# hrz2000/CustomNeRF

Hardware: AMD Instinct MI355X
Metric: training rays/s (higher is better)
Workload: dtype f16

## Files before the change

customnerf_amd/csrc/field.hip:

```cpp
#include "field_common.h"

template <bool H>
__device__ __forceinline__ void fld_stage_all(typename Prec<H>::elem_t *lds, const FieldDims &dm, const FieldLds &lo, const float *__restrict__ pnet,
                                              const float *__restrict__ pden, const float *__restrict__ prgb, bool with_rgb,
                                              uint32_t i0 = threadIdx.x, uint32_t istride = FLD_THREADS) {
    using P = Prec<H>;
    const uint32_t S64 = FLD_HID / P::KS, Senc = dm.enc_pad / P::KS;
    const float *n0 = pnet, *n1 = pnet + FLD_HID * dm.enc_pad;
    const float *n2 = n1 + (dm.n_hidden_geo == 2 ? FLD_HID * FLD_HID : 0);
    fld_stage_layer<H, 0>(lds + lo.off[0], n0, FLD_HID, dm.enc_pad, 2, Senc, dm.enc_pad, i0, istride);
    if (dm.n_hidden_geo == 2) fld_stage_layer<H, 1>(lds + lo.off[1], n1, FLD_HID, FLD_HID, 2, S64, FLD_HID, i0, istride);
    fld_stage_layer<H, 1>(lds + lo.off[2], n2, FLD_HID, FLD_HID, 2, S64, FLD_HID, i0, istride);
    fld_stage_layer<H, 1>(lds + lo.off[3], pden, FLD_HID, FLD_HID, 2, S64, FLD_HID, i0, istride);
    fld_stage_layer<H, 1>(lds + lo.off[4], pden + FLD_HID * FLD_HID, 16, FLD_HID, 1, S64, FLD_HID, i0, istride);
    if (with_rgb) {
        const uint32_t in_r0 = FLD_HID + FLD_DIR;
        fld_stage_layer<H, 2>(lds + lo.off[5], prgb, FLD_HID, in_r0, 2, in_r0 / P::KS, in_r0, i0, istride);
        fld_stage_layer<H, 1>(lds + lo.off[6], prgb + FLD_HID * in_r0, 16, FLD_HID, 1, S64, FLD_HID, i0, istride);
    }
}

__global__ void __launch_bounds__(FLD_THREADS) k_field_pack(_Float16 *__restrict__ img, FieldDims dm, const float *__restrict__ pnet,
                                                            const float *__restrict__ pden, const float *__restrict__ prgb) {
    const FieldLds lo = fld_lds_layout<true>(dm);
    fld_stage_all<true>(img, dm, lo, pnet, pden, prgb, true, blockIdx.x * FLD_THREADS + threadIdx.x, gridDim.x * FLD_THREADS);
}
__device__ __forceinline__ void fld_copy_image(_Float16 *lds, const void *__restrict__ img, uint32_t n_halves) {
    const uint4 *src = reinterpret_cast<const uint4 *>(img);
    uint4 *dst = reinterpret_cast<uint4 *>(lds);
    for (uint32_t c = threadIdx.x; c < n_halves / 8; c += FLD_THREADS) dst[c] = src[c];
}

template <bool H, bool RELU>
__device__ __forceinline__ void fld_c_to_b(const cn_f16v (&acc)[2], typename Prec<H>::frag_t *b) {
    using P = Prec<H>;
#pragma unroll
    for (int u = 0; u < 2; u++) {
#pragma unroll
        for (int sub = 0; sub < P::FR; sub++) {
            if constexpr (H) {
                union { cn_h8 h; cn_h2 p[4]; } f;
#pragma unroll
                for (int j = 0; j < 4; j++) {
                    cn_h2 v = {(_Float16)acc[u][8 * sub + 2 * j], (_Float16)acc[u][8 * sub + 2 * j + 1]};
                    if (RELU) v = __builtin_elementwise_max(v, cn_h2{(_Float16)0, (_Float16)0});
                    f.p[j] = v;
                }
                b[u * P::FR + sub] = f.h;
            } else {
                float v = acc[u][sub];
                if (RELU) v = fmaxf(v, 0.0f);
                b[u * P::FR + sub] = v;
            }
        }
    }
}

template <bool H>
__device__ __forceinline__ void fld_dir_frags(const float *__restrict__ dirs, uint32_t dir_group, uint32_t p, bool valid, uint32_t hi,
                                              typename Prec<H>::frag_t *b) {
    float dx = 0, dy = 0, dz = 0;
    if (valid) {
        const float *d = dirs + (size_t)(p / dir_group) * 3;
        dx = d[0]; dy = d[1]; dz = d[2];
    }
    fld_dir_frags_from<H>(dx, dy, dz, true, hi, b);
}

__device__ __forceinline__ float fld_round_half(float v) { return (float)(_Float16)v; }

template <bool H, int SENC, int NGEO>
__global__ void __launch_bounds__(FLD_THREADS, H ? 2 : 1) k_field_fwd(const void *__restrict__ enc, const float *__restrict__ xyz, const float *__restrict__ dirs,
                                                           uint32_t dir_group, uint32_t P_, FieldDims dm, const float *__restrict__ pnet,
                                                           const float *__restrict__ pden, const float *__restrict__ prgb,
                                                           float *__restrict__ sigma, float *__restrict__ rgbc, uint32_t enc_stride,
                                                           const void *__restrict__ wimg) {
    using PR = Prec<H>;
    using frag_t = typename PR::frag_t;
    extern __shared__ __attribute__((aligned(16))) unsigned char fld_lds[];
    typename PR::elem_t *wl = reinterpret_cast<typename PR::elem_t *>(fld_lds);
    const FieldLds lo = fld_lds_layout<H>(dm);
    const bool with_rgb = rgbc != nullptr;
#ifdef CNERF_TUNING
    const bool nostage = (dir_group >> 31) != 0;
    dir_group &= 0x7FFFFFFFu;
    if (nostage) { fld_stage_all<H>(wl, dm, lo, pnet, pden, prgb, with_rgb); __syncthreads(); }
#endif
    if constexpr (H) {
        if (wimg) fld_copy_image(wl, wimg, with_rgb ? lo.off[7] : lo.off[5]);
        else fld_stage_all<H>(wl, dm, lo, pnet, pden, prgb, with_rgb);
    } else {
        fld_stage_all<H>(wl, dm, lo, pnet, pden, prgb, with_rgb);
    }
    __syncthreads();

    const uint32_t lane = threadIdx.x & 63, wave = threadIdx.x >> 6, hi = lane >> 5;
    constexpr uint32_t S64 = FLD_HID / PR::KS, SDIR = FLD_DIR / PR::KS;
    const uint32_t n_tiles = (P_ + FLD_TILE - 1) / FLD_TILE;
    unsigned char *dir_scratch = fld_lds + lo.off[7] * sizeof(typename PR::elem_t) + wave * 64;
    const bool dir_uniform = H && (dir_group % FLD_TILE) == 0;
    for (uint32_t tile = blockIdx.x * FLD_WAVES + wave; tile < n_tiles; tile += gridDim.x * FLD_WAVES) {
        asm volatile("" ::: "memory");
        const uint32_t p = tile * FLD_TILE + (lane & 31);
        const bool valid = p < P_;

        frag_t x0[SENC];
        fld_load_enc<H, SENC>(enc, enc_stride, dm.L, p, valid, hi, x0);

        cn_f16v acc[2];
        frag_t h[2 * PR::FR];
        fld_zero(acc);
        fld_gemm<H, 2, SENC>(wl + lo.off[0], SENC, 0, x0, lane, acc);
        fld_c_to_b<H, true>(acc, h);
        if (NGEO == 2) {
            fld_zero(acc);
            fld_gemm<H, 2, S64>(wl + lo.off[1], S64, 0, h, lane, acc);
            fld_c_to_b<H, true>(acc, h);
        }
        frag_t fea[2 * PR::FR];
        fld_zero(acc);
        fld_gemm<H, 2, S64>(wl + lo.off[2], S64, 0, h, lane, acc);
        fld_c_to_b<H, false>(acc, fea);

        fld_zero(acc);
        fld_gemm<H, 2, S64>(wl + lo.off[3], S64, 0, fea, lane, acc);
        fld_c_to_b<H, true>(acc, h);
        cn_f16v out[1];
        fld_zero(out);
        fld_gemm<H, 1, S64>(wl + lo.off[4], S64, 0, h, lane, out);
        if (valid && hi == 0) {
            float raw = out[0][0];
            if (H) raw = fld_round_half(raw);
            const float x = xyz[(size_t)p * 3], y = xyz[(size_t)p * 3 + 1], z = xyz[(size_t)p * 3 + 2];
            const float g = H ? 5.0f * __expf(-(x * x + y * y + z * z) * (1.0f / 0.08f)) : 5.0f * expf(-(x * x + y * y + z * z) / 0.08f);
            sigma[p] = H ? __expf(raw + g) : expf(raw + g);
        }

        if (with_rgb) {
            frag_t dfr[SDIR];
            if constexpr (H) {
                if (dir_uniform) {
                    const float *dp = dirs + (size_t)(__builtin_amdgcn_readfirstlane(tile) * FLD_TILE / dir_group) * 3;
                    fld_dir_frags_uniform(dp[0], dp[1], dp[2], lane, hi, dir_scratch, dfr);
                } else {
                    fld_dir_frags<H>(dirs, dir_group, p, valid, hi, dfr);
                }
            } else {
                fld_dir_frags<H>(dirs, dir_group, p, valid, hi, dfr);
            }
            constexpr uint32_t SR0 = S64 + SDIR;
            fld_zero(acc);
            fld_gemm<H, 2, S64>(wl + lo.off[5], SR0, 0, fea, lane, acc);
            fld_gemm<H, 2, SDIR>(wl + lo.off[5], SR0, S64, dfr, lane, acc);
            fld_c_to_b<H, true>(acc, h);
            fld_zero(out);
            fld_gemm<H, 1, S64>(wl + lo.off[6], S64, 0, h, lane, out);
            if (valid && hi == 0) {
                float o4[4];
#pragma unroll
                for (int k = 0; k < 4; k++) {
                    float v = H ? __builtin_amdgcn_rcpf(1.0f + __expf(-out[0][k])) : 1.0f / (1.0f + expf(-out[0][k]));
                    if (H) v = fld_round_half(v);
                    o4[k] = (k < (int)dm.n_rgb_out) ? v : 0.0f;
                }
                *reinterpret_cast<float4 *>(rgbc + (size_t)p * 4) = make_float4(o4[0], o4[1], o4[2], o4[3]);
            }
        }
    }
}

template <bool H>
static int fld_launch_fwd(const void *enc, const float *xyz, const float *dirs, uint32_t dir_group, uint32_t P_, const FieldDims &dm,
                          const float *pnet, const float *pden, const float *prgb, float *sigma, float *rgbc, hipStream_t st, uint32_t enc_stride,
                          const void *wimg) {
    const FieldLds lo = fld_lds_layout<H>(dm);
    const uint32_t lds_bytes = lo.off[7] * sizeof(typename Prec<H>::elem_t) + FLD_WAVES * 64;
    const uint32_t n_tiles = cn_div_up(P_, FLD_TILE);
    uint32_t blocks = cn_div_up(n_tiles, FLD_WAVES);
    const uint32_t max_blocks = H ? 768 : 256;
    if (blocks > max_blocks) blocks = max_blocks;
#ifdef CNERF_TUNING
    static const int nostage = cn_tune_env("CNERF_FLD_NOSTAGE", 0);
    if (nostage) dir_group |= 0x80000000u;
#endif
    const bool ok = fld_dispatch(dm, [&](auto se16, auto ng) {
        auto kern = k_field_fwd<H, se16 * 16 / Prec<H>::KS, ng>;
        (void)hipFuncSetAttribute(reinterpret_cast<const void *>(kern), hipFuncAttributeMaxDynamicSharedMemorySize, lds_bytes);
        hipLaunchKernelGGL(kern, dim3(blocks), dim3(FLD_THREADS), lds_bytes, st, enc, xyz, dirs, dir_group, P_, dm, pnet, pden, prgb, sigma, rgbc, enc_stride, wimg);
    });
    if (!ok) return CNERF_EINVAL;
    return cn_launch_status();
}

extern "C" {

int cnerf_field_weight_image_bytes(uint32_t enc_dim, uint32_t n_hidden_geo, uint32_t n_rgb_out, uint64_t *bytes) {
    FieldDims dm;
    int rc = fld_dims(enc_dim, n_hidden_geo, n_rgb_out, dm);
    if (rc) return rc;
    if (!bytes) return CNERF_ENULL;
    *bytes = (uint64_t)fld_lds_layout<true>(dm).off[7] * sizeof(_Float16);
    return CNERF_OK;
}

int cnerf_field_pack_weights(uint32_t enc_dim, uint32_t n_hidden_geo, uint32_t n_rgb_out, const float *params_net, const float *params_den,
                             const float *params_rgb, void *image, uint64_t image_bytes, void *stream) {
    FieldDims dm;
    int rc = fld_dims(enc_dim, n_hidden_geo, n_rgb_out, dm);
    if (rc) return rc;
    if (!params_net || !params_den || !params_rgb || !image) return CNERF_ENULL;
    const uint32_t n = fld_lds_layout<true>(dm).off[7];
    if ((((uintptr_t)image) & 15) || image_bytes < (uint64_t)n * sizeof(_Float16)) return CNERF_EINVAL;
    hipLaunchKernelGGL(k_field_pack, dim3(cn_div_up(n, 4 * FLD_THREADS)), dim3(FLD_THREADS), 0, CN_STREAM(stream), reinterpret_cast<_Float16 *>(image), dm,
                       params_net, params_den, params_rgb);
    return cn_launch_status();
}

int cnerf_field_forward_img(const void *enc, const float *xyz, const float *dirs, uint32_t dir_group, uint32_t P_, uint32_t enc_dim,
                            uint32_t n_hidden_geo, uint32_t n_rgb_out, const float *params_net, const float *params_den, const float *params_rgb,
                            float *sigma, float *rgbc, int dtype, uint32_t enc_level_stride, const void *weight_image, void *stream) {
    FieldDims dm;
    int rc = fld_dims(enc_dim, n_hidden_geo, n_rgb_out, dm);
    if (rc) return rc;
    if (dtype != CNERF_F32 && dtype != CNERF_F16) return CNERF_EINVAL;
    if (dtype != CNERF_F16) weight_image = nullptr;
    if (((uintptr_t)weight_image) & 15) return CNERF_EINVAL;
    if (enc_level_stride == 0) enc_level_stride = P_;
    if (enc_level_stride < P_) return CNERF_EINVAL;
    if (P_ == 0) return CNERF_OK;
    if (!enc || !xyz || !params_net || !params_den || !sigma) return CNERF_ENULL;
    if (rgbc && (!dirs || !params_rgb || dir_group == 0)) return CNERF_ENULL;
    if (rgbc && (((uintptr_t)rgbc) & 15)) return CNERF_EINVAL;
    if (dtype == CNERF_F16)
        return fld_launch_fwd<true>(enc, xyz, dirs, dir_group, P_, dm, params_net, params_den, params_rgb, sigma, rgbc, CN_STREAM(stream), enc_level_stride,
                                    weight_image);
    return fld_launch_fwd<false>(enc, xyz, dirs, dir_group, P_, dm, params_net, params_den, params_rgb, sigma, rgbc, CN_STREAM(stream), enc_level_stride,
                                 nullptr);
}

int cnerf_field_forward_strided(const void *enc, const float *xyz, const float *dirs, uint32_t dir_group, uint32_t P_, uint32_t enc_dim,
                                uint32_t n_hidden_geo, uint32_t n_rgb_out, const float *params_net, const float *params_den, const float *params_rgb,
                                float *sigma, float *rgbc, int dtype, uint32_t enc_level_stride, void *stream) {
    return cnerf_field_forward_img(enc, xyz, dirs, dir_group, P_, enc_dim, n_hidden_geo, n_rgb_out, params_net, params_den, params_rgb, sigma, rgbc, dtype,
                                   enc_level_stride, nullptr, stream);
}

int cnerf_field_forward(const void *enc, const float *xyz, const float *dirs, uint32_t dir_group, uint32_t P_, uint32_t enc_dim,
                        uint32_t n_hidden_geo, uint32_t n_rgb_out, const float *params_net, const float *params_den, const float *params_rgb,
                        float *sigma, float *rgbc, int dtype, void *stream) {
    return cnerf_field_forward_strided(enc, xyz, dirs, dir_group, P_, enc_dim, n_hidden_geo, n_rgb_out, params_net, params_den, params_rgb, sigma, rgbc, dtype,
                                       P_, stream);
}

}
```

Measured before the change: 8.914 million.

## Process two point tiles per wave in field forward to reuse weight fragments

The forward field kernel now has each wave handle NT tiles at once (two when the encoding is f16 and small). Each weight fragment read from LDS feeds MFMAs for both tiles, and all global inputs (encoding, xyz, dirs) are loaded up front with clamped indices so their latency overlaps. This cuts LDS weight traffic per point and exposes more independent MFMA work. In exchange it doubles accumulator and fragment register use, which may lower occupancy, and it halves the number of wave work items at the same grid cap.

```diff
diff --git a/customnerf_amd/csrc/field.hip b/customnerf_amd/csrc/field.hip
--- a/customnerf_amd/csrc/field.hip
+++ b/customnerf_amd/csrc/field.hip
@@ -56,18 +56,74 @@
     }
 }
 
-template <bool H>
-__device__ __forceinline__ void fld_dir_frags(const float *__restrict__ dirs, uint32_t dir_group, uint32_t p, bool valid, uint32_t hi,
-                                              typename Prec<H>::frag_t *b) {
-    float dx = 0, dy = 0, dz = 0;
-    if (valid) {
-        const float *d = dirs + (size_t)(p / dir_group) * 3;
-        dx = d[0]; dy = d[1]; dz = d[2];
-    }
-    fld_dir_frags_from<H>(dx, dy, dz, true, hi, b);
-}
-
 __device__ __forceinline__ float fld_round_half(float v) { return (float)(_Float16)v; }
+
+template <bool H, int SENC>
+struct FldTileIn {
+    typename std::conditional<H, uint32_t, float>::type e[H ? 4 * SENC : SENC];
+    float x[3], d[3];
+};
+
+template <bool H, int SENC>
+__device__ __forceinline__ void fld_load_tile(const void *__restrict__ enc, uint32_t enc_stride, uint32_t L, const float *__restrict__ xyz,
+                                              const float *__restrict__ dirs, uint32_t dir_group, uint32_t tile, uint32_t n_tiles, uint32_t P_,
+                                              uint32_t lane, FldTileIn<H, SENC> &in) {
+    const uint32_t hi = lane >> 5;
+    const uint32_t tc = tile < n_tiles ? tile : n_tiles - 1;
+    const uint32_t pl = tc * FLD_TILE + (lane & 31), pc = pl < P_ ? pl : P_ - 1;
+    if constexpr (H) {
+        const uint32_t *e = reinterpret_cast<const uint32_t *>(enc);
+#pragma unroll
+        for (int i = 0; i < 4 * SENC; i++) {
+            const uint32_t level = 8 * (i >> 2) + 4 * hi + (i & 3);
+            in.e[i] = e[(size_t)(level < L ? level : L - 1) * enc_stride + pc];
+        }
+    } else {
+        const float *e = reinterpret_cast<const float *>(enc);
+#pragma unroll
+        for (int s = 0; s < SENC; s++) {
+            const uint32_t feat = 2 * s + hi, level = feat >> 1;
+            in.e[s] = e[((size_t)(level < L ? level : L - 1) * enc_stride + pc) * 2 + (feat & 1)];
+        }
+    }
+#pragma unroll
+    for (int c = 0; c < 3; c++) in.x[c] = xyz[(size_t)pc * 3 + c];
+    const float *d = dirs ? dirs + (size_t)(pc / dir_group) * 3 : xyz;
+#pragma unroll
+    for (int c = 0; c < 3; c++) in.d[c] = d[c];
+}
+
+template <bool H, int SENC>
+__device__ __forceinline__ void fld_enc_frags(const FldTileIn<H, SENC> &in, uint32_t L, bool valid, uint32_t hi, typename Prec<H>::frag_t (&b)[SENC]) {
+    if constexpr (H) {
+#pragma unroll
+        for (int s = 0; s < SENC; s++) {
+            union { cn_h8 h; uint32_t u[4]; } f;
+#pragma unroll
+            for (int jj = 0; jj < 4; jj++) f.u[jj] = (valid && 8 * s + 4 * hi + jj < L) ? in.e[4 * s + jj] : 0u;
+            b[s] = f.h;
+        }
+    } else {
+#pragma unroll
+        for (int s = 0; s < SENC; s++) b[s] = (valid && ((2 * s + hi) >> 1) < L) ? in.e[s] : 0.0f;
+    }
+}
+
+template <bool H, int NT, int T, int NS, int NB>
+__device__ __forceinline__ void fld_gemm_nt(const typename Prec<H>::elem_t *wf, uint32_t S, uint32_t s0, const typename Prec<H>::frag_t (&b)[NT][NB],
+                                            uint32_t lane, cn_f16v (&acc)[NT][T]) {
+#pragma unroll
+    for (int s = 0; s < NS; s++) {
+#pragma unroll
+        for (int t = 0; t < T; t++) {
+            const typename Prec<H>::frag_t a = fld_load_frag<H>(wf, t, S, s0 + s, lane);
+#pragma unroll
+            for (int k = 0; k < NT; k++) acc[k][t] = Prec<H>::mfma(a, b[k][s], acc[k][t]);
+        }
+    }
+}
+
+template <bool H, int SENC> constexpr int FLD_FWD_TILES = (H && SENC <= 2) ? 2 : 1;
 
 template <bool H, int SENC, int NGEO>
 __global__ void __launch_bounds__(FLD_THREADS, H ? 2 : 1) k_field_fwd(const void *__restrict__ enc, const float *__restrict__ xyz, const float *__restrict__ dirs,
@@ -77,6 +133,7 @@
                                                            const void *__restrict__ wimg) {
     using PR = Prec<H>;
     using frag_t = typename PR::frag_t;
+    constexpr int NT = FLD_FWD_TILES<H, SENC>;
     extern __shared__ __attribute__((aligned(16))) unsigned char fld_lds[];
     typename PR::elem_t *wl = reinterpret_cast<typename PR::elem_t *>(fld_lds);
     const FieldLds lo = fld_lds_layout<H>(dm);
@@ -96,74 +153,102 @@
 
     const uint32_t lane = threadIdx.x & 63, wave = threadIdx.x >> 6, hi = lane >> 5;
     constexpr uint32_t S64 = FLD_HID / PR::KS, SDIR = FLD_DIR / PR::KS;
-    const uint32_t n_tiles = (P_ + FLD_TILE - 1) / FLD_TILE;
-    unsigned char *dir_scratch = fld_lds + lo.off[7] * sizeof(typename PR::elem_t) + wave * 64;
+    const uint32_t n_tiles = (P_ + FLD_TILE - 1) / FLD_TILE, n_groups = (n_tiles + NT - 1) / NT;
+    unsigned char *dir_scratch = fld_lds + lo.off[7] * sizeof(typename PR::elem_t) + wave * NT * 64;
     const bool dir_uniform = H && (dir_group % FLD_TILE) == 0;
-    for (uint32_t tile = blockIdx.x * FLD_WAVES + wave; tile < n_tiles; tile += gridDim.x * FLD_WAVES) {
+    const float *dirs_in = with_rgb ? dirs : nullptr;
+    for (uint32_t g = blockIdx.x * FLD_WAVES + wave; g < n_groups; g += gridDim.x * FLD_WAVES) {
         asm volatile("" ::: "memory");
-        const uint32_t p = tile * FLD_TILE + (lane & 31);
-        const bool valid = p < P_;
-
-        frag_t x0[SENC];
-        fld_load_enc<H, SENC>(enc, enc_stride, dm.L, p, valid, hi, x0);
-
-        cn_f16v acc[2];
-        frag_t h[2 * PR::FR];
-        fld_zero(acc);
-        fld_gemm<H, 2, SENC>(wl + lo.off[0], SENC, 0, x0, lane, acc);
-        fld_c_to_b<H, true>(acc, h);
+        FldTileIn<H, SENC> in[NT];
+        uint32_t p[NT];
+        bool valid[NT];
+        frag_t x0[NT][SENC];
+#pragma unroll
+        for (int k = 0; k < NT; k++) {
+            const uint32_t tile = g * NT + k;
+            p[k] = tile * FLD_TILE + (lane & 31);
+            valid[k] = tile < n_tiles && p[k] < P_;
+            fld_load_tile<H, SENC>(enc, enc_stride, dm.L, xyz, dirs_in, dir_group, tile, n_tiles, P_, lane, in[k]);
+        }
+#pragma unroll
+        for (int k = 0; k < NT; k++) fld_enc_frags<H, SENC>(in[k], dm.L, valid[k], hi, x0[k]);
+
+        cn_f16v acc[NT][2];
+        frag_t h[NT][2 * PR::FR];
+#pragma unroll
+        for (int k = 0; k < NT; k++) fld_zero(acc[k]);
+        fld_gemm_nt<H, NT, 2, SENC>(wl + lo.off[0], SENC, 0, x0, lane, acc);
+#pragma unroll
+        for (int k = 0; k < NT; k++) fld_c_to_b<H, true>(acc[k], h[k]);
         if (NGEO == 2) {
-            fld_zero(acc);
-            fld_gemm<H, 2, S64>(wl + lo.off[1], S64, 0, h, lane, acc);
-            fld_c_to_b<H, true>(acc, h);
-        }
-        frag_t fea[2 * PR::FR];
-        fld_zero(acc);
-        fld_gemm<H, 2, S64>(wl + lo.off[2], S64, 0, h, lane, acc);
-        fld_c_to_b<H, false>(acc, fea);
-
-        fld_zero(acc);
-        fld_gemm<H, 2, S64>(wl + lo.off[3], S64, 0, fea, lane, acc);
-        fld_c_to_b<H, true>(acc, h);
-        cn_f16v out[1];
-        fld_zero(out);
-        fld_gemm<H, 1, S64>(wl + lo.off[4], S64, 0, h, lane, out);
-        if (valid && hi == 0) {
-            float raw = out[0][0];
-            if (H) raw = fld_round_half(raw);
-            const float x = xyz[(size_t)p * 3], y = xyz[(size_t)p * 3 + 1], z = xyz[(size_t)p * 3 + 2];
-            const float g = H ? 5.0f * __expf(-(x * x + y * y + z * z) * (1.0f / 0.08f)) : 5.0f * expf(-(x * x + y * y + z * z) / 0.08f);
-            sigma[p] = H ? __expf(raw + g) : expf(raw + g);
+#pragma unroll
+            for (int k = 0; k < NT; k++) fld_zero(acc[k]);
+            fld_gemm_nt<H, NT, 2, S64>(wl + lo.off[1], S64, 0, h, lane, acc);
+#pragma unroll
+            for (int k = 0; k < NT; k++) fld_c_to_b<H, true>(acc[k], h[k]);
+        }
+        frag_t fea[NT][2 * PR::FR];
+#pragma unroll
+        for (int k = 0; k < NT; k++) fld_zero(acc[k]);
+        fld_gemm_nt<H, NT, 2, S64>(wl + lo.off[2], S64, 0, h, lane, acc);
+#pragma unroll
+        for (int k = 0; k < NT; k++) fld_c_to_b<H, false>(acc[k], fea[k]);
+
+#pragma unroll
+        for (int k = 0; k < NT; k++) fld_zero(acc[k]);
+        fld_gemm_nt<H, NT, 2, S64>(wl + lo.off[3], S64, 0, fea, lane, acc);
+#pragma unroll
+        for (int k = 0; k < NT; k++) fld_c_to_b<H, true>(acc[k], h[k]);
+        cn_f16v out[NT][1];
+#pragma unroll
+        for (int k = 0; k < NT; k++) fld_zero(out[k]);
+        fld_gemm_nt<H, NT, 1, S64>(wl + lo.off[4], S64, 0, h, lane, out);
+#pragma unroll
+        for (int k = 0; k < NT; k++) {
+            if (valid[k] && hi == 0) {
+                float raw = out[k][0][0];
+                if (H) raw = fld_round_half(raw);
+                const float x = in[k].x[0], y = in[k].x[1], z = in[k].x[2];
+                const float gb = H ? 5.0f * __expf(-(x * x + y * y + z * z) * (1.0f / 0.08f)) : 5.0f * expf(-(x * x + y * y + z * z) / 0.08f);
+                sigma[p[k]] = H ? __expf(raw + gb) : expf(raw + gb);
+            }
         }
 
         if (with_rgb) {
-            frag_t dfr[SDIR];
-            if constexpr (H) {
-                if (dir_uniform) {
-                    const float *dp = dirs + (size_t)(__builtin_amdgcn_readfirstlane(tile) * FLD_TILE / dir_group) * 3;
-                    fld_dir_frags_uniform(dp[0], dp[1], dp[2], lane, hi, dir_scratch, dfr);
-                } else {
-                    fld_dir_frags<H>(dirs, dir_group, p, valid, hi, dfr);
+            frag_t dfr[NT][SDIR];
+#pragma unroll
+            for (int k = 0; k < NT; k++) {
+                bool uniform = false;
+                if constexpr (H) {
+                    if (dir_uniform) {
+                        fld_dir_frags_uniform(in[k].d[0], in[k].d[1], in[k].d[2], lane, hi, dir_scratch + 64 * k, dfr[k]);
+                        uniform = true;
+                    }
                 }
-            } else {
-                fld_dir_frags<H>(dirs, dir_group, p, valid, hi, dfr);
+                if (!uniform) fld_dir_frags_from<H>(valid[k] ? in[k].d[0] : 0.0f, valid[k] ? in[k].d[1] : 0.0f, valid[k] ? in[k].d[2] : 0.0f, true, hi, dfr[k]);
             }
             constexpr uint32_t SR0 = S64 + SDIR;
-            fld_zero(acc);
-            fld_gemm<H, 2, S64>(wl + lo.off[5], SR0, 0, fea, lane, acc);
-            fld_gemm<H, 2, SDIR>(wl + lo.off[5], SR0, S64, dfr, lane, acc);
-            fld_c_to_b<H, true>(acc, h);
-            fld_zero(out);
-            fld_gemm<H, 1, S64>(wl + lo.off[6], S64, 0, h, lane, out);
-            if (valid && hi == 0) {
-                float o4[4];
-#pragma unroll
-                for (int k = 0; k < 4; k++) {
-                    float v = H ? __builtin_amdgcn_rcpf(1.0f + __expf(-out[0][k])) : 1.0f / (1.0f + expf(-out[0][k]));
-                    if (H) v = fld_round_half(v);
-                    o4[k] = (k < (int)dm.n_rgb_out) ? v : 0.0f;
+#pragma unroll
+            for (int k = 0; k < NT; k++) fld_zero(acc[k]);
+            fld_gemm_nt<H, NT, 2, S64>(wl + lo.off[5], SR0, 0, fea, lane, acc);
+            fld_gemm_nt<H, NT, 2, SDIR>(wl + lo.off[5], SR0, S64, dfr, lane, acc);
+#pragma unroll
+            for (int k = 0; k < NT; k++) fld_c_to_b<H, true>(acc[k], h[k]);
+#pragma unroll
+            for (int k = 0; k < NT; k++) fld_zero(out[k]);
+            fld_gemm_nt<H, NT, 1, S64>(wl + lo.off[6], S64, 0, h, lane, out);
+#pragma unroll
+            for (int k = 0; k < NT; k++) {
+                if (valid[k] && hi == 0) {
+                    float o4[4];
+#pragma unroll
+                    for (int c = 0; c < 4; c++) {
+                        float v = H ? __builtin_amdgcn_rcpf(1.0f + __expf(-out[k][0][c])) : 1.0f / (1.0f + expf(-out[k][0][c]));
+                        if (H) v = fld_round_half(v);
+                        o4[c] = (c < (int)dm.n_rgb_out) ? v : 0.0f;
+                    }
+                    *reinterpret_cast<float4 *>(rgbc + (size_t)p[k] * 4) = make_float4(o4[0], o4[1], o4[2], o4[3]);
                 }
-                *reinterpret_cast<float4 *>(rgbc + (size_t)p * 4) = make_float4(o4[0], o4[1], o4[2], o4[3]);
             }
         }
     }
@@ -174,17 +259,18 @@
                           const float *pnet, const float *pden, const float *prgb, float *sigma, float *rgbc, hipStream_t st, uint32_t enc_stride,
                           const void *wimg) {
     const FieldLds lo = fld_lds_layout<H>(dm);
-    const uint32_t lds_bytes = lo.off[7] * sizeof(typename Prec<H>::elem_t) + FLD_WAVES * 64;
     const uint32_t n_tiles = cn_div_up(P_, FLD_TILE);
-    uint32_t blocks = cn_div_up(n_tiles, FLD_WAVES);
     const uint32_t max_blocks = H ? 768 : 256;
-    if (blocks > max_blocks) blocks = max_blocks;
 #ifdef CNERF_TUNING
     static const int nostage = cn_tune_env("CNERF_FLD_NOSTAGE", 0);
     if (nostage) dir_group |= 0x80000000u;
 #endif
     const bool ok = fld_dispatch(dm, [&](auto se16, auto ng) {
-        auto kern = k_field_fwd<H, se16 * 16 / Prec<H>::KS, ng>;
+        constexpr int SENC = se16 * 16 / Prec<H>::KS, NT = FLD_FWD_TILES<H, SENC>;
+        const uint32_t lds_bytes = lo.off[7] * sizeof(typename Prec<H>::elem_t) + FLD_WAVES * NT * 64;
+        uint32_t blocks = cn_div_up(cn_div_up(n_tiles, NT), FLD_WAVES);
+        if (blocks > max_blocks) blocks = max_blocks;
+        auto kern = k_field_fwd<H, SENC, ng>;
         (void)hipFuncSetAttribute(reinterpret_cast<const void *>(kern), hipFuncAttributeMaxDynamicSharedMemorySize, lds_bytes);
         hipLaunchKernelGGL(kern, dim3(blocks), dim3(FLD_THREADS), lds_bytes, st, enc, xyz, dirs, dir_group, P_, dm, pnet, pden, prgb, sigma, rgbc, enc_stride, wimg);
     });
```

After: 8.929 million, median of 6. About the same (+0.2%).
